# karenyang/GCN-VAE

Measured on AMD Instinct MI355X. Metric: edges/sec R-GCN forward+backward, FB15k-237 emb=200, higher is better.
Workload: dtype f32; 1 GPU; FB15k-237-shaped synthetic full graph (BASELINE configs[1]): 14541 entities, 474 directed relation types, E=544230 directed edges on this rank (544230 in the trained graph), 2-layer R-GCN-VAE bdd num_bases=100 emb_dim=200 dropout 0.2, 0 IAF blocks, DistMult decoder on T=220000 triplets per rank, step = fwd + loss(BCE+reg+KL+MMD) + bwd + clip + Adam; edges_per_gpu=544230, trained_graph_edges=544230, nodes=14541, triplets_per_gpu=220000, n_flows=0, gemm_precision=f32, launch=hipgraph, parallelism=single GPU, optimizer=replicated clip + Adam, k1_operands=f32

## Files before the change

gcn-vae_amd/csrc/k_loss.hip:

```cpp
#include "common.h"

namespace gv {

constexpr int RED_BLOCKS = 1024;

__device__ __forceinline__ float block_sum_256(float v, float* sm ) {
    v = wave_sum(v);
    const int lane = threadIdx.x & 63, w = threadIdx.x >> 6;
    __syncthreads();
    if (lane == 0) sm[w] = v;
    __syncthreads();
    return sm[0] + sm[1] + sm[2] + sm[3];
}

__global__ __launch_bounds__(256) void k_final_sum(const float* part, int n, float scale, float* out, int accumulate) {
    __shared__ float sm[4];
    float acc = 0.f;
    for (int i = threadIdx.x; i < n; i += 256) acc += part[i];
    const float tot = block_sum_256(acc, sm);
    if (threadIdx.x == 0) *out = accumulate ? *out + scale * tot : scale * tot;
}

__global__ __launch_bounds__(256) void k_loss_combine(const float* p0, int n0, float s0, const float* p1, int n1, float s1,
                                                      const float* p2, int n2, float s2, const float* p3, int n3, float s3,
// ... 754 lines not shown
__global__ __launch_bounds__(1024) void k_kl_bwd_mix_final(const float* part, const float* z_pre, const float* gkl,
                                                           float gscale, float* g_zpre, int accumulate, int64_t n, int h,
                                                           int k, int nsl, const int* rows_dev) {
    __shared__ float sm[64][16];
    const int total = 2 * k * h, kh = k * h;
    const int i = blockIdx.x * 16 + (threadIdx.x & 15);
    float acc = sum_slices_16x64(part, total, nsl, i, sm);
    if ((threadIdx.x >> 4) != 0 || i >= total) return;
    const float cg = gscale * (gkl ? *gkl : 1.f) / (float)(rows_dev ? (int64_t)*rows_dev : n);
    if (i >= kh) {
        const float raw = z_pre[i];
        acc *= raw > 20.f ? 1.f : 1.f / (1.f + expf(-raw));
    }
    g_zpre[i] = accumulate ? g_zpre[i] + cg * acc : cg * acc;
}

constexpr int MMD_WAVES = 16;

template <int CPL>
__device__ __forceinline__ void mmd_load_row(const float* p, int h, int lane, float (&v)[CPL]) {
#pragma unroll
    for (int i = 0; i < CPL; ++i) v[i] = (lane + 64 * i < h) ? p[lane + 64 * i] : 0.f;
}

template <int CPL>
__device__ __forceinline__ float mmd_d2(const float (&a)[CPL], const float (&b)[CPL]) {
    float d2 = 0.f;
#pragma unroll
    for (int i = 0; i < CPL; ++i) { const float d = a[i] - b[i]; d2 = fmaf(d, d, d2); }
    return d2;
}

template <int CPL>
__global__ __launch_bounds__(64 * MMD_WAVES) void k_mmd_fwd(const float* x, const float* y, const int64_t* yidx, int sx, int sy,
                                                             int h, float* part) {
    __shared__ float sm[MMD_WAVES];
    const int lane = threadIdx.x & 63, w = threadIdx.x >> 6;
    const bool is_x = (int)blockIdx.x < sx;
    auto row_of = [&](bool from_y, int j) -> const float* {
        return from_y ? y + (size_t)(yidx ? yidx[j] : j) * h : x + (size_t)j * h;
    };
    float av[CPL];
    mmd_load_row<CPL>(row_of(!is_x, is_x ? (int)blockIdx.x : (int)blockIdx.x - sx), h, lane, av);
    const float inv = 1.f / ((float)h * (float)h);
    float tot = 0.f;
    for (int pass = 0; pass < (is_x ? 2 : 1); ++pass) {
        const bool b_is_y = pass == 0 ? !is_x : true;
        const int nb = pass == 0 ? (is_x ? sx : sy) : sy;
        const float wt = pass == 0 ? 1.f / ((float)nb * (float)nb) : -2.f / ((float)sx * (float)sy);
        for (int j = w; j < nb; j += 4 * MMD_WAVES) {
            float b0[CPL], b1[CPL], b2[CPL], b3[CPL];
            const int j1 = j + MMD_WAVES, j2 = j + 2 * MMD_WAVES, j3 = j + 3 * MMD_WAVES;
            mmd_load_row<CPL>(row_of(b_is_y, j), h, lane, b0);
            mmd_load_row<CPL>(row_of(b_is_y, min(j1, nb - 1)), h, lane, b1);
            mmd_load_row<CPL>(row_of(b_is_y, min(j2, nb - 1)), h, lane, b2);
            mmd_load_row<CPL>(row_of(b_is_y, min(j3, nb - 1)), h, lane, b3);
            const float d0 = wave_sum(mmd_d2<CPL>(av, b0)), d1 = wave_sum(mmd_d2<CPL>(av, b1));
            const float d2 = wave_sum(mmd_d2<CPL>(av, b2)), d3 = wave_sum(mmd_d2<CPL>(av, b3));
            tot += wt * expf(-d0 * inv);
            if (j1 < nb) tot += wt * expf(-d1 * inv);
            if (j2 < nb) tot += wt * expf(-d2 * inv);
            if (j3 < nb) tot += wt * expf(-d3 * inv);
        }
    }
    if (lane == 0) sm[w] = tot;
    __syncthreads();
    if (threadIdx.x == 0) {
        float s = 0.f;
#pragma unroll
        for (int i = 0; i < MMD_WAVES; ++i) s += sm[i];
        part[blockIdx.x] = s;
    }
}

template <int CPL>
__global__ __launch_bounds__(64 * MMD_WAVES) void k_mmd_bwd(const float* x, const float* y, const int64_t* yidx, int sx, int sy,
                                                             int h, const float* gmmd, float gscale, float* gx, float* gy) {
    __shared__ float sm[MMD_WAVES][64 * CPL];
    const int lane = threadIdx.x & 63, w = threadIdx.x >> 6;
    const bool is_x = (int)blockIdx.x < sx;
    const int row = is_x ? blockIdx.x : blockIdx.x - sx;
    auto row_of = [&](bool from_y, int j) -> const float* {
        return from_y ? y + (size_t)(yidx ? yidx[j] : j) * h : x + (size_t)j * h;
    };
    float av[CPL], acc[CPL];
    mmd_load_row<CPL>(row_of(!is_x, row), h, lane, av);
#pragma unroll
    for (int i = 0; i < CPL; ++i) acc[i] = 0.f;
    const float inv = 1.f / ((float)h * (float)h);
    const float g = gscale * (gmmd ? *gmmd : 1.f);
    const int n_same = is_x ? sx : sy, n_other = is_x ? sy : sx;
    const float c_same = g * (-2.f * inv) * 2.f / ((float)n_same * (float)n_same);
    const float c_other = g * (-2.f * inv) * (-2.f) / ((float)sx * (float)sy);
    for (int pass = 0; pass < 2; ++pass) {
        const bool b_is_y = pass == 0 ? !is_x : is_x;
        const int nb = pass == 0 ? n_same : n_other;
        const float cf = pass == 0 ? c_same : c_other;
        for (int j = w; j < nb; j += 2 * MMD_WAVES) {
            float b0[CPL], b1[CPL];
            const int j1 = j + MMD_WAVES;
            mmd_load_row<CPL>(row_of(b_is_y, j), h, lane, b0);
            mmd_load_row<CPL>(row_of(b_is_y, min(j1, nb - 1)), h, lane, b1);
            const float d0 = wave_sum(mmd_d2<CPL>(av, b0)), d1 = wave_sum(mmd_d2<CPL>(av, b1));
            const float k0 = cf * expf(-d0 * inv), k1 = j1 < nb ? cf * expf(-d1 * inv) : 0.f;
#pragma unroll
            for (int i = 0; i < CPL; ++i) acc[i] = fmaf(k0, av[i] - b0[i], fmaf(k1, av[i] - b1[i], acc[i]));
        }
    }
#pragma unroll
    for (int i = 0; i < CPL; ++i) sm[w][lane + 64 * i] = acc[i];
    __syncthreads();
    const bool indexed = !is_x && yidx;
    float* o = is_x ? gx + (size_t)row * h : gy + (size_t)(yidx ? yidx[row] : row) * h;
    for (int c = threadIdx.x; c < h; c += 64 * MMD_WAVES) {
        float s = 0.f;
#pragma unroll
        for (int i = 0; i < MMD_WAVES; ++i) s += sm[i][c];
        if (indexed) atomicAdd(o + c, s);
        else o[c] = s;
    }
}

__device__ __forceinline__ float rl_dyn(float v, int src_lane) { return __shfl(v, src_lane); }

template <int G>
__device__ __forceinline__ void mmd_load_row4(const float* p, const bool (&on)[G], const int (&col)[G], float4 (&v)[G]) {
#pragma unroll
    for (int g = 0; g < G; ++g) v[g] = on[g] ? *reinterpret_cast<const float4*>(p + col[g]) : make_float4(0.f, 0.f, 0.f, 0.f);
}
template <int G>
__device__ __forceinline__ float mmd_d2_4(const float4 (&a)[G], const float4 (&b)[G]) {
    float d2 = 0.f;
#pragma unroll
    for (int g = 0; g < G; ++g) {
        const float d0 = a[g].x - b[g].x, d1 = a[g].y - b[g].y, d2_ = a[g].z - b[g].z, d3 = a[g].w - b[g].w;
        d2 = fmaf(d0, d0, d2); d2 = fmaf(d1, d1, d2); d2 = fmaf(d2_, d2_, d2); d2 = fmaf(d3, d3, d2);
    }
    return d2;
}

template <int G>
__global__ __launch_bounds__(64 * MMD_WAVES) void k_mmd_fwd_g(const float* x, const float* y, const int64_t* yidx, int sx, int sy,
                                                               int h, float* part) {
    __shared__ float sm[MMD_WAVES];
    const int lane = threadIdx.x & 63, l16 = lane & 15, w = threadIdx.x >> 6;
    const int grp = (int)(threadIdx.x >> 4);
    constexpr int NG = 4 * MMD_WAVES;
    const bool is_x = (int)blockIdx.x < sx;
    auto row_of = [&](bool from_y, int j) -> const float* {
        return from_y ? y + (size_t)(yidx ? yidx[j] : j) * h : x + (size_t)j * h;
    };
    bool on[G];
    int col[G];
#pragma unroll
    for (int g = 0; g < G; ++g) { col[g] = 4 * (l16 + 16 * g); on[g] = col[g] < h; }
    float4 av[G];
    mmd_load_row4<G>(row_of(!is_x, is_x ? (int)blockIdx.x : (int)blockIdx.x - sx), on, col, av);
    const float inv = 1.f / ((float)h * (float)h);
    float tot = 0.f;
    for (int pass = 0; pass < (is_x ? 2 : 1); ++pass) {
        const bool b_is_y = pass == 0 ? !is_x : true;
        const int nb = pass == 0 ? (is_x ? sx : sy) : sy;
        const float wt = pass == 0 ? 1.f / ((float)nb * (float)nb) : -2.f / ((float)sx * (float)sy);
        for (int j0 = 0; j0 < nb; j0 += 2 * NG) {
            const int j = j0 + grp, j1 = j + NG;
            float4 b0[G], b1[G];
            mmd_load_row4<G>(row_of(b_is_y, min(j, nb - 1)), on, col, b0);
            mmd_load_row4<G>(row_of(b_is_y, min(j1, nb - 1)), on, col, b1);
            const float d0 = row16_sum(mmd_d2_4<G>(av, b0)), d1 = row16_sum(mmd_d2_4<G>(av, b1));
            if (j < nb) tot += wt * expf(-d0 * inv);
            if (j1 < nb) tot += wt * expf(-d1 * inv);
        }
    }
    const float t = (rl_bcast_f(tot, 0) + rl_bcast_f(tot, 16)) + (rl_bcast_f(tot, 32) + rl_bcast_f(tot, 48));
    if (lane == 0) sm[w] = t;
    __syncthreads();
    if (threadIdx.x == 0) {
        float s = 0.f;
#pragma unroll
        for (int i = 0; i < MMD_WAVES; ++i) s += sm[i];
        part[blockIdx.x] = s;
    }
}

template <int G>
__global__ __launch_bounds__(64 * MMD_WAVES) void k_mmd_bwd_g(const float* x, const float* y, const int64_t* yidx, int sx, int sy,
                                                               int h, const float* gmmd, float gscale, float* gx, float* gy) {
    __shared__ float4 sm[MMD_WAVES][16 * G];
    const int lane = threadIdx.x & 63, l16 = lane & 15, w = threadIdx.x >> 6;
    const int grp = (int)(threadIdx.x >> 4);
    constexpr int NG = 4 * MMD_WAVES;
    const bool is_x = (int)blockIdx.x < sx;
    const int row = is_x ? blockIdx.x : blockIdx.x - sx;
    auto row_of = [&](bool from_y, int j) -> const float* {
        return from_y ? y + (size_t)(yidx ? yidx[j] : j) * h : x + (size_t)j * h;
    };
    bool on[G];
    int col[G];
#pragma unroll
    for (int g = 0; g < G; ++g) { col[g] = 4 * (l16 + 16 * g); on[g] = col[g] < h; }
    float4 av[G], acc[G];
    mmd_load_row4<G>(row_of(!is_x, row), on, col, av);
#pragma unroll
    for (int g = 0; g < G; ++g) acc[g] = make_float4(0.f, 0.f, 0.f, 0.f);
    const float inv = 1.f / ((float)h * (float)h);
    const float gg = gscale * (gmmd ? *gmmd : 1.f);
    const int n_same = is_x ? sx : sy, n_other = is_x ? sy : sx;
    const float c_same = gg * (-2.f * inv) * 2.f / ((float)n_same * (float)n_same);
    const float c_other = gg * (-2.f * inv) * (-2.f) / ((float)sx * (float)sy);
    for (int pass = 0; pass < 2; ++pass) {
        const bool b_is_y = pass == 0 ? !is_x : is_x;
        const int nb = pass == 0 ? n_same : n_other;
        const float cf = pass == 0 ? c_same : c_other;
        for (int j0 = 0; j0 < nb; j0 += 2 * NG) {
            const int j = j0 + grp, j1 = j + NG;
            float4 b0[G], b1[G];
            mmd_load_row4<G>(row_of(b_is_y, min(j, nb - 1)), on, col, b0);
            mmd_load_row4<G>(row_of(b_is_y, min(j1, nb - 1)), on, col, b1);
            const float d0 = row16_sum(mmd_d2_4<G>(av, b0)), d1 = row16_sum(mmd_d2_4<G>(av, b1));
            const float k0 = j < nb ? cf * expf(-d0 * inv) : 0.f, k1 = j1 < nb ? cf * expf(-d1 * inv) : 0.f;
#pragma unroll
            for (int g = 0; g < G; ++g) {
                acc[g].x = fmaf(k0, av[g].x - b0[g].x, fmaf(k1, av[g].x - b1[g].x, acc[g].x));
                acc[g].y = fmaf(k0, av[g].y - b0[g].y, fmaf(k1, av[g].y - b1[g].y, acc[g].y));
                acc[g].z = fmaf(k0, av[g].z - b0[g].z, fmaf(k1, av[g].z - b1[g].z, acc[g].z));
                acc[g].w = fmaf(k0, av[g].w - b0[g].w, fmaf(k1, av[g].w - b1[g].w, acc[g].w));
            }
        }
    }
#pragma unroll
    for (int g = 0; g < G; ++g) {
        float4 t;
        t.x = (rl_dyn(acc[g].x, l16) + rl_dyn(acc[g].x, 16 + l16)) + (rl_dyn(acc[g].x, 32 + l16) + rl_dyn(acc[g].x, 48 + l16));
        t.y = (rl_dyn(acc[g].y, l16) + rl_dyn(acc[g].y, 16 + l16)) + (rl_dyn(acc[g].y, 32 + l16) + rl_dyn(acc[g].y, 48 + l16));
        t.z = (rl_dyn(acc[g].z, l16) + rl_dyn(acc[g].z, 16 + l16)) + (rl_dyn(acc[g].z, 32 + l16) + rl_dyn(acc[g].z, 48 + l16));
        t.w = (rl_dyn(acc[g].w, l16) + rl_dyn(acc[g].w, 16 + l16)) + (rl_dyn(acc[g].w, 32 + l16) + rl_dyn(acc[g].w, 48 + l16));
        if (lane < 16) sm[w][l16 + 16 * g] = t;
    }
    __syncthreads();
    const bool indexed = !is_x && yidx;
    float* o = is_x ? gx + (size_t)row * h : gy + (size_t)(yidx ? yidx[row] : row) * h;
    for (int q = threadIdx.x; q < (h >> 2); q += 64 * MMD_WAVES) {
        float4 s4 = sm[0][q];
#pragma unroll
        for (int i = 1; i < MMD_WAVES; ++i) { const float4 t = sm[i][q]; s4.x += t.x; s4.y += t.y; s4.z += t.z; s4.w += t.w; }
        if (indexed) {
            atomicAdd(o + 4 * q, s4.x); atomicAdd(o + 4 * q + 1, s4.y); atomicAdd(o + 4 * q + 2, s4.z); atomicAdd(o + 4 * q + 3, s4.w);
        } else {
            *reinterpret_cast<float4*>(o + 4 * q) = s4;
        }
    }
}

__global__ __launch_bounds__(256) void k_prior_sample_fwd(const float* z_pre, const float* eps, float* out, int s, int k, int h) {
    const int total = s * h;
    for (int i = blockIdx.x * 256 + threadIdx.x; i < total; i += gridDim.x * 256) {
        const int r = i / h, c = i - r * h, j = r % k;
        const float v = softplus_t(z_pre[(size_t)(k + j) * h + c]) + 1e-8f;
        out[i] = z_pre[(size_t)j * h + c] + eps[i] * sqrtf(v);
    }
}

__global__ __launch_bounds__(256) void k_prior_sample_bwd(const float* z_pre, const float* eps, const float* g, float* gz_pre,
                                                          int accumulate, int s, int k, int h) {
    const int total = k * h;
    for (int i = blockIdx.x * 256 + threadIdx.x; i < total; i += gridDim.x * 256) {
        const int j = i / h, c = i - j * h;
        const float raw = z_pre[(size_t)(k + j) * h + c];
        const float v = softplus_t(raw) + 1e-8f;
        float gm = 0.f, gs = 0.f;
        for (int r = j; r < s; r += k) {
            gm += g[(size_t)r * h + c];
            gs += g[(size_t)r * h + c] * eps[(size_t)r * h + c];
        }
        const float gr = gs * 0.5f / sqrtf(v) * (raw > 20.f ? 1.f : 1.f / (1.f + expf(-raw)));
        gz_pre[i] = accumulate ? gz_pre[i] + gm : gm;
        gz_pre[total + i] = accumulate ? gz_pre[total + i] + gr : gr;
    }
}

struct DmFusedParams {
    const int4* items;
    int n_items;
    const int* rel_s;
    const int* rel_o;
    const int* rel_tid;
    const float* e;
    int ld_e;
    const float* w;
    int ld_w;
    const float* labels;
    const float* bias;
    const int* pos3;
    float* score;
    float* delta;
    float* u;
    float* partial;
    float* part;
    int h;
};

constexpr int DM_PART = RED_BLOCKS;

__device__ __forceinline__ int dm_rl_i(int v, int lane) { return __builtin_amdgcn_readlane(v, lane); }

template <int U>
__global__ __launch_bounds__(256) void k_distmult_bce_fwd_grad(const DmFusedParams a) {
    __shared__ float sm[4];
    const int lane = threadIdx.x & 63, wv = threadIdx.x >> 6;
    const bool active = lane * 4 < a.h;
    const int c0 = active ? lane * 4 : 0;
    const float bv = a.bias ? *a.bias : 0.f;
    const float* __restrict__ ebase = a.e + c0;
    float lsum = 0.f, dsum = 0.f;
    auto triplet = [&](const float (&xs)[4], const float (&xo)[4], const float (&wr)[4], float y, float (&acc)[4], float& x,
                       float& d) {
        float p[4];
#pragma unroll
        for (int i = 0; i < 4; ++i) p[i] = active ? xs[i] * xo[i] : 0.f;
        float dot = p[0] * wr[0];
        dot = fmaf(p[1], wr[1], dot);
        dot = fmaf(p[2], wr[2], dot);
        dot = fmaf(p[3], wr[3], dot);
        x = wave_sum(dot) + bv;
        d = 1.f / (1.f + expf(-x)) - y;
#pragma unroll
        for (int i = 0; i < 4; ++i) acc[i] = fmaf(d, p[i], acc[i]);
    };
    for (int quad = blockIdx.x; quad * 4 < a.n_items; quad += gridDim.x) {
        const int item = __builtin_amdgcn_readfirstlane(quad * 4 + wv);
        if (item >= a.n_items) continue;
        const int4 it = a.items[item];
        if (it.x < 0) continue;
        if (it.w >= 0 && !a.partial) continue;
        float wr[4] = {0.f, 0.f, 0.f, 0.f}, acc[4] = {0.f, 0.f, 0.f, 0.f};
        if (active) load_vec<4>(a.w + (size_t)it.x * a.ld_w + c0, wr);
        for (int e0 = it.y; e0 < it.z; e0 += 64) {
            const int cnt = min(64, it.z - e0);
            int my_s = 0, my_o = 0, my_t = 0;
            float my_y = 0.f, my_x = 0.f, my_d = 0.f;
            if (lane < cnt) {
                my_s = a.rel_s[e0 + lane];
                my_o = a.rel_o[e0 + lane];
                my_t = a.rel_tid[e0 + lane];
                my_y = a.labels[my_t];
            }
            int j = 0;
            for (; j + U <= cnt; j += U) {
                float xs[U][4], xo[U][4];
#pragma unroll
                for (int u = 0; u < U; ++u) {
                    const int s = dm_rl_i(my_s, j + u), o = dm_rl_i(my_o, j + u);
                    if (active) {
                        load_vec<4>(ebase + (size_t)s * a.ld_e, xs[u]);
                        load_vec<4>(ebase + (size_t)o * a.ld_e, xo[u]);
                    }
                }
#pragma unroll
                for (int u = 0; u < U; ++u) {
                    float x, d;
                    triplet(xs[u], xo[u], wr, rl_bcast_f(my_y, j + u), acc, x, d);
                    if (lane == j + u) { my_x = x; my_d = d; }
                }
            }
            for (; j < cnt; ++j) {
                float xs[4], xo[4], x, d;
                const int s = dm_rl_i(my_s, j), o = dm_rl_i(my_o, j);
                if (active) {
                    load_vec<4>(ebase + (size_t)s * a.ld_e, xs);
                    load_vec<4>(ebase + (size_t)o * a.ld_e, xo);
                }
                triplet(xs, xo, wr, rl_bcast_f(my_y, j), acc, x, d);
                if (lane == j) { my_x = x; my_d = d; }
            }
            if (lane < cnt) {
                a.score[my_t] = my_x;
                if (a.pos3) {
                    a.delta[a.pos3[3 * (size_t)my_t]] = my_d;
                    a.delta[a.pos3[3 * (size_t)my_t + 1]] = my_d;
                } else {
                    a.delta[my_t] = my_d;
                }
                lsum += fmaxf(my_x, 0.f) - my_x * my_y + log1pf(expf(-fabsf(my_x)));
                dsum += my_d;
            }
        }
        if (active) store_vec<4>((it.w >= 0 ? a.partial + (size_t)it.w * a.h : a.u + (size_t)it.x * a.h) + c0, acc);
    }
    const float lt = block_sum_256(lsum, sm);
    const float dt = block_sum_256(dsum, sm);
    if (threadIdx.x == 0) {
        a.part[blockIdx.x] = lt;
        a.part[DM_PART + blockIdx.x] = dt;
    }
}

struct DmFinishParams {
    const float* gloss;
    const float* u;
    const float* partial;
    const int4* fix;
    int n_fix;
    const int* rowptr;
    int chunk, num_rels, h;
    const float* w;
    int ld_w;
    float reg_scale;
    float* g_w;
    int ld_gw, accumulate;
    const float* delta;
    float* d_out;
    int64_t n_coef;
    const float* part;
    int n_part;
    float* dbias;
    int64_t t;
    int nb_rows, nb_coef;
};

__global__ __launch_bounds__(256) void k_distmult_grad_finish(const DmFinishParams a) {
    __shared__ float sm[4];
    const float g = a.gloss ? *a.gloss : 1.f;
    const float gt = g / (float)a.t;
    const int b = blockIdx.x;
    if (b < a.nb_rows) {
        const int lane = threadIdx.x & 63;
        const int n_rows = a.num_rels + a.n_fix;
        const int row = b * 4 + (threadIdx.x >> 6);
        if (row >= n_rows || lane * 4 >= a.h) return;
        const int c0 = lane * 4;
        int r;
        float acc[4];
        if (row < a.num_rels) {
            r = row;
            if (a.rowptr[r + 1] - a.rowptr[r] > a.chunk) return;
            load_vec<4>(a.u + (size_t)r * a.h + c0, acc);
        } else {
            const int4 f = a.fix[row - a.num_rels];
            if (f.x < 0) return;
            r = f.x;
            const float4* __restrict__ p = reinterpret_cast<const float4*>(a.partial + (size_t)f.y * a.h + c0);
            const size_t stride = (size_t)(a.h >> 2);
            float4 s[4];
#pragma unroll
            for (int i = 0; i < 4; ++i) s[i] = make_float4(0.f, 0.f, 0.f, 0.f);
            int k = 0;
            for (; k + 4 <= f.z; k += 4) {
                float4 v[4];
#pragma unroll
                for (int i = 0; i < 4; ++i) v[i] = p[(size_t)(k + i) * stride];
#pragma unroll
                for (int i = 0; i < 4; ++i) { s[i].x += v[i].x; s[i].y += v[i].y; s[i].z += v[i].z; s[i].w += v[i].w; }
            }
            for (; k < f.z; ++k) {
                const float4 v = p[(size_t)k * stride];
                s[0].x += v.x; s[0].y += v.y; s[0].z += v.z; s[0].w += v.w;
            }
            acc[0] = (s[0].x + s[1].x) + (s[2].x + s[3].x);
            acc[1] = (s[0].y + s[1].y) + (s[2].y + s[3].y);
            acc[2] = (s[0].z + s[1].z) + (s[2].z + s[3].z);
            acc[3] = (s[0].w + s[1].w) + (s[2].w + s[3].w);
        }
        float wr[4], out[4];
        load_vec<4>(a.w + (size_t)r * a.ld_w + c0, wr);
        float* o = a.g_w + (size_t)r * a.ld_gw + c0;
        if (a.accumulate) load_vec<4>(o, out);
#pragma unroll
        for (int i = 0; i < 4; ++i) {
            const float v = fmaf(gt, acc[i], g * a.reg_scale * wr[i]);
            out[i] = a.accumulate ? out[i] + v : v;
        }
        store_vec<4>(o, out);
    } else if (b < a.nb_rows + a.nb_coef) {
        for (int64_t i = (int64_t)(b - a.nb_rows) * 256 + threadIdx.x; i < a.n_coef; i += (int64_t)a.nb_coef * 256)
            a.d_out[i] = gt * a.delta[i];
    } else {
        float acc = 0.f;
        for (int i = threadIdx.x; i < a.n_part; i += 256) acc += a.part[DM_PART + i];
        const float tot = block_sum_256(acc, sm);
        if (threadIdx.x == 0) *a.dbias = gt * tot;
    }
}

constexpr int KL_SLICES = 256;
constexpr int KL_FUSED_KT = 16;

}

using namespace gv;

#define GV_ST ((hipStream_t)stream)

static int red_blocks(int64_t n, int per_block) {
    int64_t b = (n + per_block - 1) / per_block;
    return (int)(b < 1 ? 1 : (b > RED_BLOCKS ? RED_BLOCKS : b));
}

static int sq2_blocks(int64_t n, int cap) {
    const int b = red_blocks(n, 4096);
    return b > cap ? cap : b;
}

static int kl_blocks(int64_t n) { return (int)((n + 3) / 4 > RED_BLOCKS ? RED_BLOCKS : (n + 3) / 4); }

extern "C" int gv_distmult_bce_fwd(const float* embed, int ld_e, const float* w_rel, int ld_w,
                                   const int32_t* triplets, const int32_t* order, const float* labels, const float* bias,
                                   float* score, float* loss, float* workspace, int64_t t, int h, void* stream) {
    GV_REQUIRE(embed && w_rel && triplets && labels && score && workspace, GV_ERR_NULL,
               "gv_distmult_bce_fwd: NULL pointer");
    GV_REQUIRE(t > 0 && h > 0 && ld_e >= h && ld_w >= h, GV_ERR_SHAPE, "gv_distmult_bce_fwd: bad shape");
    const int nb = red_blocks(t, 16);
    hipLaunchKernelGGL(k_distmult_bce, dim3(nb), dim3(256), 0, GV_ST, embed, ld_e, w_rel, ld_w, triplets, order, labels,
                       bias, score, workspace, t, h);
    if (loss) hipLaunchKernelGGL(k_final_sum, dim3(1), dim3(256), 0, GV_ST, workspace, nb, 1.f / (float)t, loss, 0);
    return launch_status("gv_distmult_bce_fwd");
}

extern "C" int gv_bce_grad(const float* score, const float* labels, const float* gloss, float* dscore,
                           const int32_t* pos3, float* dscore_inc, float* dscore_rel, float* dbias, float* workspace,
                           int64_t t, void* stream) {
    GV_REQUIRE(score && labels && dscore && workspace, GV_ERR_NULL, "gv_bce_grad: NULL pointer");
    GV_REQUIRE(!pos3 || (dscore_inc && dscore_rel), GV_ERR_NULL, "gv_bce_grad: pos3 needs dscore_inc and dscore_rel");
    GV_REQUIRE(t > 0, GV_ERR_SHAPE, "gv_bce_grad: t=%lld", (long long)t);
    const int nb = red_blocks(t, 256);
    hipLaunchKernelGGL(k_bce_grad, dim3(nb), dim3(256), 0, GV_ST, score, labels, gloss, dscore, pos3, dscore_inc,
                       dscore_rel, workspace, t);
    if (dbias) hipLaunchKernelGGL(k_final_sum, dim3(1), dim3(256), 0, GV_ST, workspace, nb, 1.f, dbias, 0);
    return launch_status("gv_bce_grad");
}

extern "C" int gv_mean_sq(const float* x, int64_t n, float scale, float* out, float* workspace, int accumulate,
                          void* stream) {
    GV_REQUIRE(x && out && workspace, GV_ERR_NULL, "gv_mean_sq: NULL pointer");
    GV_REQUIRE(n > 0, GV_ERR_SHAPE, "gv_mean_sq: n=%lld", (long long)n);
    const int nb = red_blocks(n, 4096);
    hipLaunchKernelGGL(k_sumsq_part, dim3(nb), dim3(256), 0, GV_ST, x, n, workspace);
    hipLaunchKernelGGL(k_final_sum, dim3(1), dim3(256), 0, GV_ST, workspace, nb, scale, out, accumulate);
    return launch_status("gv_mean_sq");
}

__global__ __launch_bounds__(256) void k_sumsq2_part(const float* x1, int64_t n1, float s1, int nb1, const float* x2,
                                                     int64_t n2, float s2, float* part, const int* rows_dev, int64_t rows_host) {
    __shared__ float sm[4];
    if (rows_dev) {
        const int64_t rows = *rows_dev;
        n1 = n1 / rows_host * rows;
        s1 *= (float)rows_host / (float)rows;
    }
    const bool first = (int)blockIdx.x < nb1;
    const float* x = first ? x1 : x2;
    const int64_t n = first ? n1 : n2;
    const int b = first ? blockIdx.x : blockIdx.x - nb1, nb = first ? nb1 : gridDim.x - nb1;
    float acc = 0.f;
    for (int64_t i = (int64_t)b * 256 + threadIdx.x; i < n; i += (int64_t)nb * 256) acc = fmaf(x[i], x[i], acc);
    const float tot = block_sum_256(acc, sm);
    if (threadIdx.x == 0) part[blockIdx.x] = tot * (first ? s1 : s2);
}

extern "C" int gv_mean_sq2(const float* x1, int64_t n1, float scale1, const float* x2, int64_t n2, float scale2, float* out,
                           float* workspace, const int32_t* rows_dev, int64_t rows_host, void* stream) {
    GV_REQUIRE(x1 && x2 && workspace, GV_ERR_NULL, "gv_mean_sq2: NULL pointer");
    GV_REQUIRE(n1 > 0 && n2 > 0, GV_ERR_SHAPE, "gv_mean_sq2: empty input");
    GV_REQUIRE(!rows_dev || (rows_host > 0 && n1 % rows_host == 0), GV_ERR_SHAPE, "gv_mean_sq2: rows_host=%lld does not divide n1",
               (long long)rows_host);
    const int nb1 = sq2_blocks(n1, 768), nb2 = sq2_blocks(n2, 255);
    hipLaunchKernelGGL(k_sumsq2_part, dim3(nb1 + nb2), dim3(256), 0, GV_ST, x1, n1, scale1, nb1, x2, n2, scale2, workspace, rows_dev,
                       rows_host);
    if (out) hipLaunchKernelGGL(k_final_sum, dim3(1), dim3(256), 0, GV_ST, workspace, nb1 + nb2, 1.f, out, 0);
    return launch_status("gv_mean_sq2");
}

extern "C" int64_t gv_kl_workspace_bytes(int64_t n, int h, int k) {
    (void)n;
    return (int64_t)sizeof(float) * (3 * (int64_t)k * h + RED_BLOCKS + (int64_t)KL_SLICES * 2 * k * h);
}

static bool kl_fwd_v4(int nb, size_t lds, hipStream_t st, const float* z, const float* m, int ld_m, const float* v, const float* mix,
                      const float* flp, float* resp, float* part, int64_t n, int h, int k, const int* rows_dev, const float* h2,
                      const float* eps, float* z_out, float* v_out, float* m_out) {
    static const int env = getenv("GV_KL_V4") ? atoi(getenv("GV_KL_V4")) : 1;
    const bool al = aligned16(mix) && (!z || aligned16(z)) && (!m || (aligned16(m) && ld_m % 4 == 0)) && (!v || aligned16(v)) &&
                    (!h2 || aligned16(h2)) && (!eps || aligned16(eps)) && (!z_out || aligned16(z_out)) && (!v_out || aligned16(v_out)) &&
                    (!m_out || aligned16(m_out));
    if (!env || h % 4 != 0 || h > 1024 || !al) return false;
    static const int v5 = getenv("GV_KL_V5") ? atoi(getenv("GV_KL_V5")) : 1;
    if (v5 && h <= (v5 == 2 ? 512 : 256) && k <= 16) {
        if (h <= 256)
            hipLaunchKernelGGL(k_kl_fwd_v5<4>, dim3(nb), dim3(256), lds, st, z, m, ld_m, v, mix, flp, resp, part, n, h, k, rows_dev, h2,
                               eps, z_out, v_out, m_out);
        else
            hipLaunchKernelGGL(k_kl_fwd_v5<8>, dim3(nb), dim3(256), lds, st, z, m, ld_m, v, mix, flp, resp, part, n, h, k, rows_dev, h2,
                               eps, z_out, v_out, m_out);
        return true;
    }
#define GV_KL_V4(G_) hipLaunchKernelGGL(k_kl_fwd_v4<G_>, dim3(nb), dim3(256), lds, st, z, m, ld_m, v, mix, flp, resp, part, n, h, k, rows_dev, h2, eps, z_out, v_out, m_out)
    if (h <= 256) GV_KL_V4(1);
    else if (h <= 512) GV_KL_V4(2);
    else GV_KL_V4(4);
#undef GV_KL_V4
    return true;
}

extern "C" int gv_kl_fwd(const float* z, const float* m, int ld_m, const float* v, const float* z_pre,
                         const float* flp, float* resp, float* kl, float* workspace, int64_t n, int h, int k,
                         const int32_t* rows_dev, void* stream) {
    GV_REQUIRE(z && m && v && z_pre && resp && workspace, GV_ERR_NULL, "gv_kl_fwd: NULL pointer");
    GV_REQUIRE(n > 0 && h > 0 && k > 0 && k <= KL_KMAX && ld_m >= h, GV_ERR_SHAPE, "gv_kl_fwd: n=%lld h=%d k=%d",
               (long long)n, h, k);
    const size_t lds = (size_t)2 * k * h * sizeof(float);
    GV_REQUIRE(lds <= 64 * 1024, GV_ERR_SHAPE, "gv_kl_fwd: mixture table %zu B exceeds the 64 KiB LDS budget", lds);
    GV_REQUIRE(!(rows_dev && kl), GV_ERR_SHAPE, "gv_kl_fwd: with rows_dev the mean is finished by gv_loss_combine (kl must be NULL)");
    float* mix = workspace;
    float* part = workspace + 3 * (size_t)k * h;
    hipLaunchKernelGGL(k_kl_mix, dim3((k * h + 255) / 256), dim3(256), 0, GV_ST, z_pre, k, h, mix);
    const int nb = kl_blocks(n);
    GV_REQUIRE(h <= 1024, GV_ERR_SHAPE, "gv_kl_fwd: h=%d > 1024 unsupported", h);
#define GV_KL_FWD(CPL_) hipLaunchKernelGGL(k_kl_fwd<CPL_>, dim3(nb), dim3(256), lds, GV_ST, z, m, ld_m, v, mix, flp, resp, part, n, h, k, rows_dev)
    if (kl_fwd_v4(nb, lds, GV_ST, z, m, ld_m, v, mix, flp, resp, part, n, h, k, rows_dev, nullptr, nullptr, nullptr, nullptr, nullptr)) {}
    else if (h <= 64) GV_KL_FWD(1);
    else if (h <= 128) GV_KL_FWD(2);
    else if (h <= 256) GV_KL_FWD(4);
    else if (h <= 512) GV_KL_FWD(8);
    else GV_KL_FWD(16);
#undef GV_KL_FWD
    if (kl) hipLaunchKernelGGL(k_final_sum, dim3(1), dim3(256), 0, GV_ST, part, nb, 1.f / (float)n, kl, 0);
    return launch_status("gv_kl_fwd");
}

static bool kl_bwd_cols4(hipStream_t st, const float* z, const float* m, int ld_m, const float* v, const float* mix, const float* resp,
                         const float* gkl, float gscale, float z_extra, float* gz, float* gm, float* gv, float* part, int64_t n, int h,
                         int k, const int* rows_dev, const float* h2, const float* eps, const float* gz_up, float* gh2) {
    static const int env = getenv("GV_KL_BWD_V4") ? atoi(getenv("GV_KL_BWD_V4")) : 1;
    const bool al = aligned16(z) && aligned16(m) && ld_m % 4 == 0 && aligned16(v) && aligned16(mix) && aligned16(part) &&
                    (!gz || aligned16(gz)) && (!gm || aligned16(gm)) && (!gv || aligned16(gv)) && (!h2 || aligned16(h2)) &&
                    (!eps || aligned16(eps)) && (!gz_up || aligned16(gz_up)) && (!gh2 || aligned16(gh2));
    if (!env || h % 4 != 0 || h > 1024 || k > 10 || !al) return false;
    const size_t lds = ((size_t)2 * k * h / 4 + (size_t)2 * KLB_KR * KLB_WAVES * 64) * sizeof(float4);
    if (lds > 128 * 1024) return false;
    static unsigned long long lds_done = 0;
    if (lds > 64 * 1024 && !raise_dynamic_lds((const void*)k_kl_bwd_cols4<10>, 128 * 1024, lds_done, "gv_kl_bwd")) return false;
#define GV_KLB(KT_) hipLaunchKernelGGL(k_kl_bwd_cols4<KT_>, dim3((h + 255) / 256, KL_SLICES), dim3(64 * KLB_WAVES), lds, st, z, m, ld_m, v, mix, resp, gkl, \
                                       gscale, z_extra, gz, gm, gv, part, n, h, k, rows_dev, h2, eps, gz_up, gh2)
    GV_KLB(10);
#undef GV_KLB
    return true;
}

extern "C" int gv_kl_bwd(const float* z, const float* m, int ld_m, const float* v, const float* z_pre,
                         const float* resp, const float* gkl, float gscale, float z_extra, float* gz, float* gm,
                         float* gv, float* g_zpre, int accumulate_zpre, float* workspace, int mix_ready, int64_t n, int h,
                         int k, const int32_t* rows_dev, void* stream) {
    GV_REQUIRE(z && m && v && z_pre && resp && gz && gm && gv && g_zpre && workspace, GV_ERR_NULL,
               "gv_kl_bwd: NULL pointer");
    GV_REQUIRE(n > 0 && h > 0 && k > 0 && k <= KL_KMAX && ld_m >= h, GV_ERR_SHAPE, "gv_kl_bwd: bad shape");
    float* mix = workspace;
    if (!mix_ready) hipLaunchKernelGGL(k_kl_mix, dim3((k * h + 255) / 256), dim3(256), 0, GV_ST, z_pre, k, h, mix);
    float* part = workspace + 3 * (size_t)k * h + RED_BLOCKS;
    if (kl_bwd_cols4(GV_ST, z, m, ld_m, v, mix, resp, gkl, gscale, z_extra, gz, gm, gv, part, n, h, k, rows_dev, nullptr, nullptr,
                     nullptr, nullptr)) {
    } else if (k <= KL_FUSED_KT) {
        hipLaunchKernelGGL(k_kl_bwd_fused<KL_FUSED_KT>, dim3((h + 63) / 64, KL_SLICES), dim3(256), 0, GV_ST, z, m, ld_m, v, mix,
                           resp, gkl, gscale, z_extra, gz, gm, gv, part, n, h, k, rows_dev);
    } else {
        GV_REQUIRE(!rows_dev, GV_ERR_SHAPE, "gv_kl_bwd: rows_dev needs k <= %d mixture components", KL_FUSED_KT);
        const size_t lds = (size_t)2 * k * h * sizeof(float);
        const int nb = (int)((n + 3) / 4 > 1024 ? 1024 : (n + 3) / 4);
        hipLaunchKernelGGL(k_kl_bwd_nodes, dim3(nb), dim3(256), lds, GV_ST, z, m, ld_m, v, mix, resp, gkl, gscale, z_extra,
                           gz, gm, gv, n, h, k);
        hipLaunchKernelGGL(k_kl_bwd_mix_part, dim3(k, (h + 63) / 64, KL_SLICES), dim3(256), 0, GV_ST, z, mix, resp, part, n,
                           h, k);
    }
    hipLaunchKernelGGL(k_kl_bwd_mix_final, dim3((2 * k * h + 15) / 16), dim3(1024), 0, GV_ST, part, z_pre, gkl,
                       gscale, g_zpre, accumulate_zpre, n, h, k, KL_SLICES, rows_dev);
    return launch_status("gv_kl_bwd");
}

extern "C" int gv_reparam_kl_fwd(const float* h2, const float* eps, const float* z_pre, float* z, float* v, float* m_out,
                                 float* resp, float* workspace, int64_t n, int h, int k, void* stream) {
    GV_REQUIRE(h2 && eps && z_pre && z && v && resp && workspace, GV_ERR_NULL, "gv_reparam_kl_fwd: NULL pointer");
    GV_REQUIRE(n > 0 && h > 0 && h <= 1024 && k > 0 && k <= KL_KMAX, GV_ERR_SHAPE, "gv_reparam_kl_fwd: n=%lld h=%d k=%d", (long long)n,
               h, k);
    const size_t lds = (size_t)2 * k * h * sizeof(float);
    GV_REQUIRE(lds <= 64 * 1024, GV_ERR_SHAPE, "gv_reparam_kl_fwd: mixture table %zu B exceeds the 64 KiB LDS budget", lds);
    float* mix = workspace;
    float* part = workspace + 3 * (size_t)k * h;
    hipLaunchKernelGGL(k_kl_mix, dim3((k * h + 255) / 256), dim3(256), 0, GV_ST, z_pre, k, h, mix);
    const int nb = kl_blocks(n);
    const float* none = nullptr;
    const int* no_rows = nullptr;
#define GV_RKL_FWD(CPL_)                                                                                                       \
    hipLaunchKernelGGL(k_kl_fwd<CPL_>, dim3(nb), dim3(256), lds, GV_ST, none, none, h, none, (const float*)mix, none, resp, part, n, h, \
                       k, no_rows, h2, eps, z, v, m_out)
    if (kl_fwd_v4(nb, lds, GV_ST, none, none, h, none, mix, none, resp, part, n, h, k, no_rows, h2, eps, z, v, m_out)) {}
    else if (h <= 64) GV_RKL_FWD(1);
    else if (h <= 128) GV_RKL_FWD(2);
    else if (h <= 256) GV_RKL_FWD(4);
    else if (h <= 512) GV_RKL_FWD(8);
    else GV_RKL_FWD(16);
#undef GV_RKL_FWD
    return launch_status("gv_reparam_kl_fwd");
}

extern "C" int gv_reparam_kl_bwd(const float* z, const float* h2, const float* v, const float* eps, const float* z_pre,
                                 const float* resp, const float* gkl, float gscale, float z_extra, const float* gz_up,
                                 float* gh2, float* g_zpre, int accumulate_zpre, float* workspace, int64_t n, int h, int k,
                                 void* stream) {
    GV_REQUIRE(z && h2 && v && eps && z_pre && resp && gh2 && g_zpre && workspace, GV_ERR_NULL, "gv_reparam_kl_bwd: NULL pointer");
    GV_REQUIRE(n > 0 && h > 0 && k > 0 && k <= KL_FUSED_KT, GV_ERR_SHAPE, "gv_reparam_kl_bwd: n=%lld h=%d k=%d (k <= %d)", (long long)n,
               h, k, KL_FUSED_KT);
    float* mix = workspace;
    float* part = workspace + 3 * (size_t)k * h + RED_BLOCKS;
    float* none = nullptr;
    const int* no_rows = nullptr;
    if (!kl_bwd_cols4(GV_ST, z, h2, 2 * h, v, mix, resp, gkl, gscale, z_extra, none, none, none, part, n, h, k, no_rows, h2, eps, gz_up,
                      gh2))
        hipLaunchKernelGGL(k_kl_bwd_fused<KL_FUSED_KT>, dim3((h + 63) / 64, KL_SLICES), dim3(256), 0, GV_ST, z, h2, 2 * h, v,
                           (const float*)mix, resp, gkl, gscale, z_extra, none, none, none, part, n, h, k, no_rows, h2, eps, gz_up, gh2);
    hipLaunchKernelGGL(k_kl_bwd_mix_final, dim3((2 * k * h + 15) / 16), dim3(1024), 0, GV_ST, (const float*)part, z_pre, gkl, gscale,
                       g_zpre, accumulate_zpre, n, h, k, KL_SLICES, no_rows);
    return launch_status("gv_reparam_kl_bwd");
}

__global__ void k_lincomb(const float* a0, float c0, const float* a1, float c1, const float* a2, float c2, const float* a3,
                          float c3, float* out) {
    if (threadIdx.x == 0 && blockIdx.x == 0) {
        float v = 0.f;
        if (a0) v += c0 * *a0;
        if (a1) v += c1 * *a1;
        if (a2) v += c2 * *a2;
        if (a3) v += c3 * *a3;
        *out = v;
    }
}

extern "C" int gv_lincomb4(const float* a0, float c0, const float* a1, float c1, const float* a2, float c2,
                           const float* a3, float c3, float* out, void* stream) {
    GV_REQUIRE(out, GV_ERR_NULL, "gv_lincomb4: NULL output");
    hipLaunchKernelGGL(k_lincomb, dim3(1), dim3(64), 0, GV_ST, a0, c0, a1, c1, a2, c2, a3, c3, out);
    return launch_status("gv_lincomb4");
}

extern "C" int gv_mmd_fwd(const float* x, const float* y, const int64_t* y_index, int sx, int sy, int h, float* mmd,
                          float* workspace, void* stream) {
    GV_REQUIRE(x && y && workspace, GV_ERR_NULL, "gv_mmd_fwd: NULL pointer");
    GV_REQUIRE(sx > 0 && sy > 0 && h > 0 && h <= 1024 && sx + sy <= RED_BLOCKS, GV_ERR_SHAPE,
               "gv_mmd_fwd: sx=%d sy=%d h=%d (need h <= 1024, sx+sy <= %d)", sx, sy, h, RED_BLOCKS);
    static const int v2 = getenv("GV_MMD_ROWS16") ? atoi(getenv("GV_MMD_ROWS16")) : 1;
    const bool al = h % 4 == 0 && aligned16(x) && aligned16(y);
    if (v2 && al && h <= 256) hipLaunchKernelGGL(k_mmd_fwd_g<4>, dim3(sx + sy), dim3(64 * MMD_WAVES), 0, GV_ST, x, y, y_index, sx, sy, h, workspace);
    else if (v2 && al && h <= 512) hipLaunchKernelGGL(k_mmd_fwd_g<8>, dim3(sx + sy), dim3(64 * MMD_WAVES), 0, GV_ST, x, y, y_index, sx, sy, h, workspace);
    else if (h <= 256) hipLaunchKernelGGL(k_mmd_fwd<4>, dim3(sx + sy), dim3(64 * MMD_WAVES), 0, GV_ST, x, y, y_index, sx, sy, h, workspace);
    else hipLaunchKernelGGL(k_mmd_fwd<16>, dim3(sx + sy), dim3(64 * MMD_WAVES), 0, GV_ST, x, y, y_index, sx, sy, h, workspace);
    if (mmd) hipLaunchKernelGGL(k_final_sum, dim3(1), dim3(256), 0, GV_ST, workspace, sx + sy, 1.f, mmd, 0);
    return launch_status("gv_mmd_fwd");
}

extern "C" int gv_loss_combine(const float* ws_pred, int64_t t, const float* ws_reg, int64_t n_embed, int64_t n_wrel,
                               const float* ws_kl, int64_t n_nodes, int h, int k, const float* ws_mmd, int sx, int sy,
                               float reg_w, float kl_w, float mmd_w, float* scal, float* loss, const int32_t* rows_dev,
                               void* stream) {
    GV_REQUIRE(ws_pred && loss, GV_ERR_NULL, "gv_loss_combine: NULL pointer");
    GV_REQUIRE(t > 0, GV_ERR_SHAPE, "gv_loss_combine: t=%lld", (long long)t);
    const int n0 = red_blocks(t, 16);
    const int n1 = ws_reg ? sq2_blocks(n_embed, 768) + sq2_blocks(n_wrel, 255) : 0;
    const int n2 = ws_kl ? kl_blocks(n_nodes) : 0;
    const int n3 = ws_mmd ? sx + sy : 0;
    const float* kl_part = ws_kl ? ws_kl + 3 * (size_t)k * h : nullptr;
    hipLaunchKernelGGL(k_loss_combine, dim3(1), dim3(256), 0, GV_ST, ws_pred, n0, 1.f / (float)t, ws_reg, n1, 1.f, kl_part,
                       n2, ws_kl ? 1.f / (float)n_nodes : 0.f, ws_mmd, n3, 1.f, reg_w, kl_w, mmd_w, scal, loss, rows_dev,
                       (float)n_nodes);
    return launch_status("gv_loss_combine");
}

extern "C" int gv_mmd_bwd(const float* x, const float* y, const int64_t* y_index, int sx, int sy, int h, const float* gmmd,
                          float gscale, float* gx, float* gy, void* stream) {
    GV_REQUIRE(x && y && gx && gy, GV_ERR_NULL, "gv_mmd_bwd: NULL pointer");
    GV_REQUIRE(sx > 0 && sy > 0 && h > 0 && h <= 1024, GV_ERR_SHAPE, "gv_mmd_bwd: bad shape");
    static const int v2 = getenv("GV_MMD_ROWS16") ? atoi(getenv("GV_MMD_ROWS16")) : 1;
    const bool al = h % 4 == 0 && aligned16(x) && aligned16(y) && aligned16(gx) && aligned16(gy);
    if (v2 && al && h <= 256) hipLaunchKernelGGL(k_mmd_bwd_g<4>, dim3(sx + sy), dim3(64 * MMD_WAVES), 0, GV_ST, x, y, y_index, sx, sy, h, gmmd, gscale, gx, gy);
    else if (h <= 256) hipLaunchKernelGGL(k_mmd_bwd<4>, dim3(sx + sy), dim3(64 * MMD_WAVES), 0, GV_ST, x, y, y_index, sx, sy, h, gmmd, gscale, gx, gy);
    else hipLaunchKernelGGL(k_mmd_bwd<16>, dim3(sx + sy), dim3(64 * MMD_WAVES), 0, GV_ST, x, y, y_index, sx, sy, h, gmmd, gscale, gx, gy);
    return launch_status("gv_mmd_bwd");
}

extern "C" int gv_prior_sample_fwd(const float* z_pre, const float* eps, float* out, int s, int k, int h, void* stream) {
    GV_REQUIRE(z_pre && eps && out, GV_ERR_NULL, "gv_prior_sample_fwd: NULL pointer");
    GV_REQUIRE(s > 0 && k > 0 && h > 0, GV_ERR_SHAPE, "gv_prior_sample_fwd: bad shape");
    hipLaunchKernelGGL(k_prior_sample_fwd, dim3((s * h + 255) / 256), dim3(256), 0, GV_ST, z_pre, eps, out, s, k, h);
    return launch_status("gv_prior_sample_fwd");
}

extern "C" int gv_prior_sample_bwd(const float* z_pre, const float* eps, const float* g, float* gz_pre, int accumulate,
                                   int s, int k, int h, void* stream) {
    GV_REQUIRE(z_pre && eps && g && gz_pre, GV_ERR_NULL, "gv_prior_sample_bwd: NULL pointer");
    GV_REQUIRE(s > 0 && k > 0 && h > 0, GV_ERR_SHAPE, "gv_prior_sample_bwd: bad shape");
    hipLaunchKernelGGL(k_prior_sample_bwd, dim3((k * h + 255) / 256), dim3(256), 0, GV_ST, z_pre, eps, g, gz_pre, accumulate, s, k, h);
    return launch_status("gv_prior_sample_bwd");
}

extern "C" int gv_distmult_bce_fwd_grad(const int32_t* items, int n_items, const int32_t* rel_s, const int32_t* rel_o,
                                        const int32_t* rel_tid, const float* embed, int ld_e, const float* w_rel, int ld_w,
                                        const float* labels, const float* bias, const int32_t* pos3, float* score,
                                        float* delta, float* u, float* partial, float* workspace, int64_t t, int h,
                                        void* stream) {
    GV_REQUIRE(items && rel_s && rel_o && rel_tid && embed && w_rel && labels && score && delta && u && workspace,
               GV_ERR_NULL, "gv_distmult_bce_fwd_grad: NULL pointer");
    GV_REQUIRE(t > 0 && t < (1ll << 30) && n_items > 0, GV_ERR_SHAPE, "gv_distmult_bce_fwd_grad: t=%lld n_items=%d",
               (long long)t, n_items);
    GV_REQUIRE(h > 0 && h <= 256 && h % 4 == 0 && ld_e >= h && ld_w >= h && ld_e % 4 == 0 && ld_w % 4 == 0, GV_ERR_SHAPE,
               "gv_distmult_bce_fwd_grad: h=%d (ld %d, %d): the fused sweep covers h <= 256, h %% 4 == 0", h, ld_e, ld_w);
    GV_REQUIRE(aligned16(embed) && aligned16(w_rel) && aligned16(u) && aligned16(partial), GV_ERR_ALIGN,
               "gv_distmult_bce_fwd_grad: 16-B alignment required");
    DmFusedParams p{(const int4*)items, n_items, rel_s, rel_o, rel_tid, embed, ld_e, w_rel, ld_w, labels, bias, pos3,
                    score, delta, u, partial, workspace, h};
    hipLaunchKernelGGL(k_distmult_bce_fwd_grad<8>, dim3(red_blocks(t, 16)), dim3(256), 0, GV_ST, p);
    return launch_status("gv_distmult_bce_fwd_grad");
}

extern "C" int gv_distmult_grad_finish(const float* gloss, const float* u, const float* partial, const int32_t* fix,
                                       int n_fix, const int32_t* rowptr, int chunk, int num_rels, int h,
                                       const float* w_rel, int ld_w, float reg_scale, float* grad_w, int ld_gw,
                                       int accumulate, const float* delta, float* d_out, int64_t n_coef,
                                       const float* workspace, float* dbias, int64_t t, void* stream) {
    GV_REQUIRE(u && rowptr && w_rel && grad_w && delta && d_out, GV_ERR_NULL, "gv_distmult_grad_finish: NULL pointer");
    GV_REQUIRE(n_fix == 0 || (fix && partial), GV_ERR_NULL, "gv_distmult_grad_finish: split rows need fix + partial");
    GV_REQUIRE(!dbias || workspace, GV_ERR_NULL, "gv_distmult_grad_finish: dbias needs the forward's workspace");
    GV_REQUIRE(t > 0 && n_coef > 0 && n_fix >= 0 && num_rels > 0 && chunk > 0, GV_ERR_SHAPE,
               "gv_distmult_grad_finish: t=%lld n_coef=%lld n_fix=%d num_rels=%d chunk=%d", (long long)t, (long long)n_coef,
               n_fix, num_rels, chunk);
    GV_REQUIRE(h > 0 && h <= 256 && h % 4 == 0 && ld_w >= h && ld_gw >= h && ld_w % 4 == 0 && ld_gw % 4 == 0, GV_ERR_SHAPE,
               "gv_distmult_grad_finish: h=%d (ld %d, %d): h <= 256, h %% 4 == 0", h, ld_w, ld_gw);
    GV_REQUIRE(aligned16(u) && aligned16(partial) && aligned16(w_rel) && aligned16(grad_w), GV_ERR_ALIGN,
               "gv_distmult_grad_finish: 16-B alignment required");
    DmFinishParams p{gloss, u, partial, (const int4*)fix, n_fix, rowptr, chunk, num_rels, h, w_rel, ld_w, reg_scale, grad_w,
                     ld_gw, accumulate, delta, d_out, n_coef, workspace, red_blocks(t, 16), dbias, t, 0, 0};
    p.nb_rows = (num_rels + n_fix + 3) / 4;
    p.nb_coef = red_blocks(n_coef, 1024);
    hipLaunchKernelGGL(k_distmult_grad_finish, dim3(p.nb_rows + p.nb_coef + (dbias ? 1 : 0)), dim3(256), 0, GV_ST, p);
    return launch_status("gv_distmult_grad_finish");
}
```

Before: 570.9 million edges/s.

## Process four triplets per wave in DistMult BCE kernel using 16-lane rows

Restructures the fused DistMult forward+grad kernel so each wave splits into four 16-lane rows, each handling a different triplet with a float4x4 slice of the embedding, instead of one triplet per 64-lane wave with 4 floats per lane. Triplet indices and labels are staged in LDS, scores go back through LDS, and the loss sums now accumulate in shared arrays. The aim is to avoid 64-lane reductions and lanes sitting idle when h=200 (only 50 of 64 lanes were active), and to put more loads in flight. The cost is a cross-row permute reduction of the accumulators at the end of each item and more register pressure.

```diff
diff --git a/gcn-vae_amd/csrc/k_loss.hip b/gcn-vae_amd/csrc/k_loss.hip
--- a/gcn-vae_amd/csrc/k_loss.hip
+++ b/gcn-vae_amd/csrc/k_loss.hip
@@ -1080,78 +1080,95 @@
 
 constexpr int DM_PART = RED_BLOCKS;
 
-__device__ __forceinline__ int dm_rl_i(int v, int lane) { return __builtin_amdgcn_readlane(v, lane); }
-
-template <int U>
+__device__ __forceinline__ float dm_perm_f(int src_lane, float v) {
+    return __int_as_float(__builtin_amdgcn_ds_bpermute(src_lane << 2, __float_as_int(v)));
+}
+__device__ __forceinline__ float dm_delta(float x, float y) { return 1.f / (1.f + expf(-x)) - y; }
+
+constexpr int DM_U = 2;
+
 __global__ __launch_bounds__(256) void k_distmult_bce_fwd_grad(const DmFusedParams a) {
+    constexpr int U = DM_U;
     __shared__ float sm[4];
+    __shared__ int4 tb[4][64];
+    __shared__ float sums[2][256];
+    constexpr int G = 4;
     const int lane = threadIdx.x & 63, wv = threadIdx.x >> 6;
-    const bool active = lane * 4 < a.h;
-    const int c0 = active ? lane * 4 : 0;
+    const int l16 = lane & 15, rw = lane >> 4;
+    bool on[G];
+#pragma unroll
+    for (int g = 0; g < G; ++g) on[g] = 4 * (l16 + 16 * g) < a.h;
     const float bv = a.bias ? *a.bias : 0.f;
-    const float* __restrict__ ebase = a.e + c0;
-    float lsum = 0.f, dsum = 0.f;
-    auto triplet = [&](const float (&xs)[4], const float (&xo)[4], const float (&wr)[4], float y, float (&acc)[4], float& x,
-                       float& d) {
-        float p[4];
-#pragma unroll
-        for (int i = 0; i < 4; ++i) p[i] = active ? xs[i] * xo[i] : 0.f;
-        float dot = p[0] * wr[0];
-        dot = fmaf(p[1], wr[1], dot);
-        dot = fmaf(p[2], wr[2], dot);
-        dot = fmaf(p[3], wr[3], dot);
-        x = wave_sum(dot) + bv;
-        d = 1.f / (1.f + expf(-x)) - y;
-#pragma unroll
-        for (int i = 0; i < 4; ++i) acc[i] = fmaf(d, p[i], acc[i]);
-    };
+    const float* __restrict__ ebase = a.e + 4 * l16;
+    sums[0][threadIdx.x] = sums[1][threadIdx.x] = 0.f;
     for (int quad = blockIdx.x; quad * 4 < a.n_items; quad += gridDim.x) {
         const int item = __builtin_amdgcn_readfirstlane(quad * 4 + wv);
         if (item >= a.n_items) continue;
         const int4 it = a.items[item];
         if (it.x < 0) continue;
         if (it.w >= 0 && !a.partial) continue;
-        float wr[4] = {0.f, 0.f, 0.f, 0.f}, acc[4] = {0.f, 0.f, 0.f, 0.f};
-        if (active) load_vec<4>(a.w + (size_t)it.x * a.ld_w + c0, wr);
+        float4 wr[G], acc[G];
+#pragma unroll
+        for (int g = 0; g < G; ++g) {
+            wr[g] = acc[g] = make_float4(0.f, 0.f, 0.f, 0.f);
+            if (on[g]) wr[g] = *reinterpret_cast<const float4*>(a.w + (size_t)it.x * a.ld_w + 4 * l16 + 64 * g);
+        }
         for (int e0 = it.y; e0 < it.z; e0 += 64) {
             const int cnt = min(64, it.z - e0);
-            int my_s = 0, my_o = 0, my_t = 0;
-            float my_y = 0.f, my_x = 0.f, my_d = 0.f;
-            if (lane < cnt) {
-                my_s = a.rel_s[e0 + lane];
-                my_o = a.rel_o[e0 + lane];
-                my_t = a.rel_tid[e0 + lane];
-                my_y = a.labels[my_t];
-            }
-            int j = 0;
-            for (; j + U <= cnt; j += U) {
-                float xs[U][4], xo[U][4];
+            if (lane < cnt)
+                tb[wv][lane] = make_int4(a.rel_s[e0 + lane], a.rel_o[e0 + lane],
+                                         __float_as_int(a.labels[a.rel_tid[e0 + lane]]), 0);
+            __builtin_amdgcn_wave_barrier();
+            for (int j = 0; j < cnt; j += 4 * U) {
+                int2 so[U];
+                float4 xs[U][G], xo[U][G];
+#pragma unroll
+                for (int u = 0; u < U; ++u) so[u] = *reinterpret_cast<const int2*>(&tb[wv][min(j + 4 * u + rw, cnt - 1)]);
 #pragma unroll
                 for (int u = 0; u < U; ++u) {
-                    const int s = dm_rl_i(my_s, j + u), o = dm_rl_i(my_o, j + u);
-                    if (active) {
-                        load_vec<4>(ebase + (size_t)s * a.ld_e, xs[u]);
-                        load_vec<4>(ebase + (size_t)o * a.ld_e, xo[u]);
+                    const float* ps = ebase + (size_t)so[u].x * a.ld_e;
+                    const float* po = ebase + (size_t)so[u].y * a.ld_e;
+#pragma unroll
+                    for (int g = 0; g < G; ++g) {
+                        if (on[g]) {
+                            xs[u][g] = *reinterpret_cast<const float4*>(ps + 64 * g);
+                            xo[u][g] = *reinterpret_cast<const float4*>(po + 64 * g);
+                        }
                     }
                 }
 #pragma unroll
                 for (int u = 0; u < U; ++u) {
-                    float x, d;
-                    triplet(xs[u], xo[u], wr, rl_bcast_f(my_y, j + u), acc, x, d);
-                    if (lane == j + u) { my_x = x; my_d = d; }
+                    float4 (&p)[G] = xs[u];
+                    const int t = j + 4 * u + rw;
+                    const float y = __int_as_float(tb[wv][min(t, cnt - 1)].z);
+                    float dot = 0.f;
+#pragma unroll
+                    for (int g = 0; g < G; ++g) {
+                        p[g].x *= xo[u][g].x; p[g].y *= xo[u][g].y; p[g].z *= xo[u][g].z; p[g].w *= xo[u][g].w;
+                        float c = fmaf(p[g].x, wr[g].x, dot);
+                        c = fmaf(p[g].y, wr[g].y, c);
+                        c = fmaf(p[g].z, wr[g].z, c);
+                        c = fmaf(p[g].w, wr[g].w, c);
+                        dot = on[g] ? c : dot;
+                    }
+                    const float x = row16_sum(dot) + bv;
+                    const float d = t < cnt ? dm_delta(x, y) : 0.f;
+#pragma unroll
+                    for (int g = 0; g < G; ++g) {
+                        acc[g].x = fmaf(d, p[g].x, acc[g].x);
+                        acc[g].y = fmaf(d, p[g].y, acc[g].y);
+                        acc[g].z = fmaf(d, p[g].z, acc[g].z);
+                        acc[g].w = fmaf(d, p[g].w, acc[g].w);
+                    }
+                    if (l16 == 0 && t < cnt) tb[wv][t].w = __float_as_int(x);
+                    __builtin_amdgcn_sched_barrier(0);
                 }
             }
-            for (; j < cnt; ++j) {
-                float xs[4], xo[4], x, d;
-                const int s = dm_rl_i(my_s, j), o = dm_rl_i(my_o, j);
-                if (active) {
-                    load_vec<4>(ebase + (size_t)s * a.ld_e, xs);
-                    load_vec<4>(ebase + (size_t)o * a.ld_e, xo);
-                }
-                triplet(xs, xo, wr, rl_bcast_f(my_y, j), acc, x, d);
-                if (lane == j) { my_x = x; my_d = d; }
-            }
+            __builtin_amdgcn_wave_barrier();
             if (lane < cnt) {
+                const float my_y = __int_as_float(tb[wv][lane].z), my_x = __int_as_float(tb[wv][lane].w);
+                const int my_t = a.rel_tid[e0 + lane];
+                const float my_d = dm_delta(my_x, my_y);
                 a.score[my_t] = my_x;
                 if (a.pos3) {
                     a.delta[a.pos3[3 * (size_t)my_t]] = my_d;
@@ -1159,14 +1176,25 @@
                 } else {
                     a.delta[my_t] = my_d;
                 }
-                lsum += fmaxf(my_x, 0.f) - my_x * my_y + log1pf(expf(-fabsf(my_x)));
-                dsum += my_d;
-            }
-        }
-        if (active) store_vec<4>((it.w >= 0 ? a.partial + (size_t)it.w * a.h : a.u + (size_t)it.x * a.h) + c0, acc);
-    }
-    const float lt = block_sum_256(lsum, sm);
-    const float dt = block_sum_256(dsum, sm);
+                sums[0][threadIdx.x] += fmaxf(my_x, 0.f) - my_x * my_y + log1pf(expf(-fabsf(my_x)));
+                sums[1][threadIdx.x] += my_d;
+            }
+            __builtin_amdgcn_wave_barrier();
+        }
+        float* out = (it.w >= 0 ? a.partial + (size_t)it.w * a.h : a.u + (size_t)it.x * a.h) + 4 * l16;
+#pragma unroll
+        for (int g = 0; g < G; ++g) {
+            float v[4] = {acc[g].x, acc[g].y, acc[g].z, acc[g].w};
+#pragma unroll
+            for (int i = 0; i < 4; ++i) {
+                v[i] += dm_perm_f(lane ^ 16, v[i]);
+                v[i] += dm_perm_f(lane ^ 32, v[i]);
+            }
+            if (rw == 0 && on[g]) store_vec<4>(out + 64 * g, v);
+        }
+    }
+    const float lt = block_sum_256(sums[0][threadIdx.x], sm);
+    const float dt = block_sum_256(sums[1][threadIdx.x], sm);
     if (threadIdx.x == 0) {
         a.part[blockIdx.x] = lt;
         a.part[DM_PART + blockIdx.x] = dt;
@@ -1592,7 +1620,7 @@
                "gv_distmult_bce_fwd_grad: 16-B alignment required");
     DmFusedParams p{(const int4*)items, n_items, rel_s, rel_o, rel_tid, embed, ld_e, w_rel, ld_w, labels, bias, pos3,
                     score, delta, u, partial, workspace, h};
-    hipLaunchKernelGGL(k_distmult_bce_fwd_grad<8>, dim3(red_blocks(t, 16)), dim3(256), 0, GV_ST, p);
+    hipLaunchKernelGGL(k_distmult_bce_fwd_grad, dim3(red_blocks(t, 16)), dim3(256), 0, GV_ST, p);
     return launch_status("gv_distmult_bce_fwd_grad");
 }
 
```

Result: faster. 577.7 million edges/s, median of 6 (+1.2%).
